# abeauvisage/uasl_motion_estimation

Measured on AMD Instinct MI355X. Metric: frames/sec + BA iter/sec, 2000 feats x 20-keyframe window, 1/2/4/8 MI355X, higher is better.
Workload: dtype u8+f32 (MI), f64 (BA); 1 GPU; config 3: 1280x720 stereo, 2000 feats, 20-keyframe window, 11x11 MI patches; frame=KLT + MI scale LM (LM, MAX_NB_ITER 10, tolerances off) + 10 BA LM iterations, parallelism=1 independent streams (one per GPU)

## Files before the change

uasl_motion_estimation_amd/csrc/ba.hip:

```cpp
#include <algorithm>
#include <cmath>
#include <cstdio>
#include <cstring>
#include <mutex>
#include <numeric>
#include <vector>
#include <hip/hip_ext.h>
#include "me_internal.hpp"
#include "ba_kernels.hpp"
#include "roster.hpp"
#include "solve_diag.hpp"
#include "me_device.hpp"

using me_dev::wave_sync;

using namespace ba;

namespace {

constexpr double kDblMin = 2.2250738585072014e-308;
constexpr double kDblEps = 2.220446049250313e-16;

template <int Ctrl>
__device__ __forceinline__ double dpp_f64(double x);
// ... 196 lines not shown
    *rho0 = s;
    *sqrt_rho1 = 1.0;
  }
}

template <bool SC1>
__device__ __forceinline__ double a_ld(const double* p) {
  if (!SC1) return *p;
  return __builtin_bit_cast(double, __hip_atomic_load(reinterpret_cast<const unsigned long long*>(p), ME_HO_LD,
                                                      __HIP_MEMORY_SCOPE_AGENT));
}
template <bool SC1>
__device__ __forceinline__ void a_st(double* p, double v) {
  if (!SC1) {
    *p = v;
    return;
  }
  __hip_atomic_store(reinterpret_cast<unsigned long long*>(p), __builtin_bit_cast(unsigned long long, v),
                     ME_HO_ST, __HIP_MEMORY_SCOPE_AGENT);
}
__device__ __forceinline__ void drain_and_barrier() {
  asm volatile("s_waitcnt vmcnt(0)" ::: "memory");
  __syncthreads();
}


constexpr int kPtBlock = 64;

#ifndef ME_LIN_SMALL
#define ME_LIN_SMALL 64
#endif
constexpr int kLinSmall = ME_LIN_SMALL, kLinSmallMaxObs = 64 * 512;
__host__ __device__ inline int lin_block(int no) { return no <= kLinSmallMaxObs ? kLinSmall : kBlock; }
template <int OD, int BLK>
__global__ __launch_bounds__(BLK) void linearize_kernel(Geo g, Bufs b) {
  __shared__ double lds[BLK / 64];
  const State* st = b.st;
  if (st->done || !st->need_lin) return;
  const int o = blockIdx.x * BLK + threadIdx.x;
  double cost = 0;
  if (o < g.no) {
    const int cur = st->cur;
    const int ci = b.cam_idx[o], pi = b.pt_idx[o];
    double r[4], Jc[24], Jp[12];
    obs_residual<OD>(g, b, o, b.cams[cur] + 6 * ci, b.pts[cur] + 3 * pi, r, Jc, Jp);
    const double s = r[0] * r[0] + r[1] * r[1] + r[2] * r[2] + r[3] * r[3];
    double rho0, sc;
    huber(s, &rho0, &sc);
    cost = 0.5 * rho0;
    for (int k = 0; k < 4; ++k) r[k] *= sc;
    for (int k = 0; k < 24; ++k) Jc[k] *= sc;
    for (int k = 0; k < 12; ++k) Jp[k] *= sc;
    const long slot = b.pos[o];
    double* X = b.obsx + slot * kObsxStride;
    X[0] = Jp[0] * Jp[0] + Jp[3] * Jp[3] + Jp[6] * Jp[6] + Jp[9] * Jp[9];
    X[1] = Jp[0] * Jp[1] + Jp[3] * Jp[4] + Jp[6] * Jp[7] + Jp[9] * Jp[10];
    X[2] = Jp[0] * Jp[2] + Jp[3] * Jp[5] + Jp[6] * Jp[8] + Jp[9] * Jp[11];
    X[3] = Jp[1] * Jp[1] + Jp[4] * Jp[4] + Jp[7] * Jp[7] + Jp[10] * Jp[10];
    X[4] = Jp[1] * Jp[2] + Jp[4] * Jp[5] + Jp[7] * Jp[8] + Jp[10] * Jp[11];
    X[5] = Jp[2] * Jp[2] + Jp[5] * Jp[5] + Jp[8] * Jp[8] + Jp[11] * Jp[11];
    for (int a = 0; a < 3; ++a) X[6 + a] = Jp[a] * r[0] + Jp[3 + a] * r[1] + Jp[6 + a] * r[2] + Jp[9 + a] * r[3];
    if (ci - g.nf >= 0) {
      double* W = b.Wo + 18 * slot;
      for (int a = 0; a < 6; ++a)
        for (int c = 0; c < 3; ++c)
          W[a * 3 + c] = Jc[a] * Jp[c] + Jc[6 + a] * Jp[3 + c] + Jc[12 + a] * Jp[6 + c] + Jc[18 + a] * Jp[9 + c];
    }
  }
  double v[1] = {cost};
  double out[1];
  block_sum<1>(v, out, lds);
  if (threadIdx.x == 0) b.part[R_COST * g.pstride + blockIdx.x] = out[0];
}

__device__ __forceinline__ bool last_arrival_wt(unsigned* cnt, unsigned expected) {
  __shared__ int slast;
  __syncthreads();
  if (threadIdx.x == 0) {
    asm volatile("s_waitcnt vmcnt(0)" ::: "memory");
    const unsigned k = __hip_atomic_fetch_add(cnt, 1u, ME_HO_RMW, __HIP_MEMORY_SCOPE_AGENT);
    slast = k == expected - 1;
    if (slast) __hip_atomic_store(cnt, 0u, __ATOMIC_RELAXED, __HIP_MEMORY_SCOPE_AGENT);
  }
  __syncthreads();
  return slast != 0;
}

__device__ void cam_reduce_body(const Geo& g, const Bufs& b, int sharded, const double* cpart, double* colnorm,
                                double* gc_raw, double* Uraw, int ci, int first, int count) {
  __shared__ double tot[27];
  __shared__ double csl[6];
  const State* st = b.st;
  const int u = threadIdx.x;
  if (u < 27) {
    double sum = 0.0;
    for (int k = 0; k < count; ++k) sum += a_ld<true>(&cpart[27 * ((long)first + k) + u]);
    tot[u] = sum;
    if (u < 21) Uraw[21 * (long)ci + u] = sum;
    else gc_raw[6 * ci + u - 21] = sum;
  }
// ... 164 lines not shown
  double d0 = A[0];
  if (!(d0 > 0)) return false;
  d0 = sqrt(d0);
  const double l10 = A[3] / d0, l20 = A[6] / d0;
  double d1 = A[4] - l10 * l10;
  if (!(d1 > 0)) return false;
  d1 = sqrt(d1);
  const double l21 = (A[7] - l20 * l10) / d1;
  double d2 = A[8] - l20 * l20 - l21 * l21;
  if (!(d2 > 0)) return false;
  d2 = sqrt(d2);
  L[0] = d0; L[1] = 0; L[2] = 0;
  L[3] = l10; L[4] = d1; L[5] = 0;
  L[6] = l20; L[7] = l21; L[8] = d2;
  return true;
}
__device__ __forceinline__ void fwd3(const double* L, const double* b, double* y) {
  y[0] = b[0] / L[0];
  y[1] = (b[1] - L[3] * y[0]) / L[4];
  y[2] = (b[2] - L[6] * y[0] - L[7] * y[1]) / L[8];
}
__device__ __forceinline__ void bwd3(const double* L, const double* y, double* x) {
  x[2] = y[2] / L[8];
  x[1] = (y[1] - L[7] * x[2]) / L[4];
  x[0] = (y[0] - L[3] * x[1] - L[6] * x[2]) / L[0];
}

constexpr int kSchurPts = 16, kSchurPtsWide = 32, kSchurPtsSmall = 8;
#ifndef ME_SCHUR_NT
#define ME_SCHUR_NT 5
#endif
constexpr int kSchurNtMax = ME_SCHUR_NT;
constexpr size_t kSchurLdsCap = 150 * 1024;
__host__ __device__ inline size_t schur_lds_bytes(int P, int Rz) { return 8 * (size_t)3 * P * Rz + 4 * 3 * (size_t)P; }

template <int W>
__device__ __forceinline__ int group_min(int x) {
  if (W >= 2) x = min(x, dpp_i32<kDppQuadSwap1>(x));
  if (W >= 4) x = min(x, dpp_i32<kDppQuadSwap2>(x));
  if (W >= 8) x = min(x, dpp_i32<kDppRowHalfMirror>(x));
  if (W >= 16) x = min(x, dpp_i32<kDppRowMirror>(x));
  if (W >= 32) x = min(x, __shfl_xor(x, 16, W));
  if (W >= 64) x = min(x, __shfl_xor(x, 32, W));
  return x;
}
template <int W>
__device__ __forceinline__ int group_max(int x) {
  if (W >= 2) x = max(x, dpp_i32<kDppQuadSwap1>(x));
  if (W >= 4) x = max(x, dpp_i32<kDppQuadSwap2>(x));
  if (W >= 8) x = max(x, dpp_i32<kDppRowHalfMirror>(x));
  if (W >= 16) x = max(x, dpp_i32<kDppRowMirror>(x));
  if (W >= 32) x = max(x, __shfl_xor(x, 16, W));
  if (W >= 64) x = max(x, __shfl_xor(x, 32, W));
  return x;
}

#ifdef ME_SCHUR_STAMPS
#define SCHUR_T(i)                                                                     \
  do {                                                                                 \
    if (sblk == 0 && threadIdx.x == 0) {                                               \
      const long long tt_ = (long long)__builtin_amdgcn_s_memtime();                   \
      if ((i) > 0) st->stamps[5 + (i)] += tt_ - sch_prev_;                             \
      sch_prev_ = tt_;                                                                 \
    }                                                                                  \
  } while (0)
#else
#define SCHUR_T(i) \
  do {             \
  } while (0)
#endif
template <int NT, int BLK, int PTS>
__global__ __launch_bounds__(BLK) void pt_schur_kernel(Geo g, Bufs b, Opts o, CamArgs ca) {
  constexpr int SL = BLK / PTS, NW = BLK / 64;
  extern __shared__ double smem[];
  __shared__ double red[8];
  if (ca.on && (int)blockIdx.x < ca.ncam) {
    if (threadIdx.x >= kBlock) return;
    const int q = blockIdx.x;
    if (q >= g.ncu) return;
#ifdef ME_EXP_NOCAM
    return;
#endif
    if (g.od == 4)
      cam_assemble_body<4>(g, b, ca.cpart, 0, ca.colnorm, ca.gc_raw, ca.Uraw, q);
    else
      cam_assemble_body<2>(g, b, ca.cpart, 0, ca.colnorm, ca.gc_raw, ca.Uraw, q);
    return;
  }
  const int sblk = (int)blockIdx.x - (ca.on ? ca.ncam : 0);
  State* st = b.st;
  if (st->done) return;
#ifdef ME_SCHUR_STAMPS
  long long sch_prev_ = 0;
  if (sblk == 0 && threadIdx.x == 0) st->stamps[12] += 1;
#endif
  SCHUR_T(0);
  const int need_lin = st->need_lin, scaled = st->scaled, cur = st->cur;
  const double* obsx = b.obsx;
  const double* Wo = b.Wo;
  const double radius = st->radius;
  const bool final_pass = st->iterations >= o.max_num_iterations;
  if (sblk == 0 && threadIdx.x == 0) st->final_pass = final_pass;
  const int P = g.spts, Rz = g.Rpad, rows = 3 * P, nks = rows / 4;
  const int sup = sblk / (8 * g.sgrp), r8 = sblk - sup * 8 * g.sgrp;
  const int run = 8 * sup + (r8 & 7), tgrp = r8 >> 3;
  if (run >= g.nruns) {
    if (need_lin && threadIdx.x == 0) b.part[R_GMAX_PT * g.pstride + sblk] = 0.0;
    return;
  }
  const int bA = g.sorted ? b.rband[2 * run] : 0, bB = g.sorted ? b.rband[2 * run + 1] : g.T - 1;
  const int nb = bB - bA + 1, ns = nb + (bB < g.T - 1 ? 1 : 0), ntile = ns * (ns + 1) / 2;
  if (tgrp * g.stpw >= ntile) {
    if (need_lin && threadIdx.x == 0) b.part[R_GMAX_PT * g.pstride + sblk] = 0.0;
    return;
  }
  const bool lead = tgrp == 0;
  double* Y = smem;
  int* band = reinterpret_cast<int*>(Y + (size_t)rows * Rz);
  const int tid = threadIdx.x, lane = tid & 63, wave = __builtin_amdgcn_readfirstlane(tid >> 6);
  const int gi = tid / SL, gl = tid & (SL - 1);
  int tI[NT], tJ[NT];
#pragma unroll
  for (int u = 0; u < NT; ++u) {
    int p = tgrp * g.stpw + wave + NW * u, ka = 0;
    if (p >= ntile) p = -1;
    int rem = p < 0 ? 0 : p;
    while (rem >= ns - ka) {
      rem -= ns - ka;
      ++ka;
    }
    const int kb = ka + rem;
    tI[u] = p < 0 ? -1 : (ka < nb ? bA + ka : g.T - 1);
    tJ[u] = p < 0 ? -1 : (kb < nb ? bA + kb : g.T - 1);
  }
  double4_t acc[NT];
#pragma unroll
  for (int u = 0; u < NT; ++u) acc[u] = double4_t{0.0, 0.0, 0.0, 0.0};
  double gm = 0;
  for (int sc = 0; sc < g.rsub; ++sc) {
    const int pos = run * g.rlen + sc * P + gi;
    const int j = pos < g.np ? (g.sorted ? b.order[pos] : pos) : g.np;
    double* Yp = Y + (size_t)(3 * gi) * Rz;
    for (int i = gl; i < 3 * Rz / 2; i += SL) reinterpret_cast<double2*>(Yp)[i] = double2{0.0, 0.0};
    if (j < g.np) {
      const int beg = b.p_off[j], end = b.p_off[j + 1];
      const int q0 = beg + gl;
      int ci0 = -1, cprev0 = -1, cnext0 = -2;
      double w0[18], cs0[6], X0[9];
      for (int i = 0; i < 9; ++i) X0[i] = 0.0;
      if (q0 < end) {
        ci0 = b.p_cam[q0];
        if (q0 > beg) cprev0 = b.p_cam[q0 - 1];
        if (q0 + 1 < end) cnext0 = b.p_cam[q0 + 1];
        if (need_lin)
          for (int i = 0; i < 9; ++i) X0[i] = obsx[(long)q0 * kObsxStride + i];
        if (ci0 >= 0) {
          for (int i = 0; i < 18; ++i) w0[i] = Wo[18 * (long)q0 + i];
          for (int a = 0; a < 6; ++a) cs0[a] = b.csc[6 * ci0 + a];
        }
      }
      double Vs[9], gs[3], pv[3], xv[3];
      if (need_lin) {
        for (int a = 0; a < 3; ++a) xv[a] = b.pts[cur][3 * (long)j + a];
        if (scaled)
          for (int a = 0; a < 3; ++a) pv[a] = b.psc[3 * (long)j + a];
        double V[9];
        for (int i = 0; i < 9; ++i) V[i] = X0[i];
        for (int q = q0 + SL; q < end; q += SL)
          for (int i = 0; i < 9; ++i) V[i] += obsx[(long)q * kObsxStride + i];
        SCHUR_T(1);
      for (int i = 0; i < 9; ++i) V[i] = group_sum<SL>(V[i]);
        if (!scaled) {
          pv[0] = g.jacobi ? 1.0 / (1.0 + sqrt(V[0])) : 1.0;
          pv[1] = g.jacobi ? 1.0 / (1.0 + sqrt(V[3])) : 1.0;
          pv[2] = g.jacobi ? 1.0 / (1.0 + sqrt(V[5])) : 1.0;
        }
        const double p0 = pv[0], p1 = pv[1], p2 = pv[2];
        Vs[0] = V[0] * p0 * p0; Vs[1] = V[1] * p0 * p1; Vs[2] = V[2] * p0 * p2;
        Vs[3] = Vs[1];          Vs[4] = V[3] * p1 * p1; Vs[5] = V[4] * p1 * p2;
        Vs[6] = Vs[2];          Vs[7] = Vs[5];          Vs[8] = V[5] * p2 * p2;
        gs[0] = V[6] * p0;
        gs[1] = V[7] * p1;
        gs[2] = V[8] * p2;
        if (gl == 0 && lead) {
          if (!scaled)
            for (int a = 0; a < 3; ++a) b.psc[3 * (long)j + a] = pv[a];
          for (int i = 0; i < 9; ++i) b.V[9 * (long)j + i] = Vs[i];
          for (int a = 0; a < 3; ++a) b.gps[3 * (long)j + a] = gs[a];
          for (int a = 0; a < 3; ++a) {
            const double xp = fmin(fmax(xv[a] - V[6 + a], g.lo[a]), g.hi[a]);
            gm = fmax(gm, fabs(xv[a] - xp));
          }
        }
      } else {
        for (int i = 0; i < 9; ++i) Vs[i] = b.V[9 * (long)j + i];
        for (int a = 0; a < 3; ++a) {
          gs[a] = b.gps[3 * (long)j + a];
          pv[a] = b.psc[3 * (long)j + a];
        }
      }
      if (!final_pass) {
      double A[9], L[9], z[3];
// ... 109 lines not shown
        auto reads = [&](const double* Yr, double* a, double* bb) {
#pragma unroll
          for (int u = 0; u < NT; ++u) {
            a[u] = Yr[cI[u]];
            bb[u] = Yr[cJ[u]];
          }
        };
        double an[NT], bn[NT];
        reads(Y0, av, bv);
#pragma unroll 1
        for (int ks = 0; ks < NKS; ks += 2) {
          reads(Y0 + (ks + 1) * kstride, an, bn);
          __builtin_amdgcn_sched_barrier(0);
          contract(ks, av, bv);
          __builtin_amdgcn_sched_barrier(0);
          reads(Y0 + min(ks + 2, NKS - 1) * kstride, av, bv);
          __builtin_amdgcn_sched_barrier(0);
          contract(ks + 1, an, bn);
          __builtin_amdgcn_sched_barrier(0);
        }
      } else {
        for (int ks = 0; ks < nks; ++ks) {
          operands(ks, av, bv);
          contract(ks, av, bv);
        }
      }
    }
    __syncthreads();
  }
  SCHUR_T(4);
  if (need_lin) {
    const double r = block_max(gm, red);
    if (tid == 0) b.part[R_GMAX_PT * g.pstride + sblk] = r;
  }
  if (final_pass) return;
#pragma unroll
  for (int u = 0; u < NT; ++u) {
    const int p = tgrp * g.stpw + wave + NW * u;
    if (p >= ntile) continue;
    double* dst = b.Spart + ((long)run * g.npairs + p) * 256;
#pragma unroll
    for (int i = 0; i < 4; ++i) dst[((lane >> 4) + 4 * i) * 16 + (lane & 15)] = acc[u][i];
  }
#ifdef ME_SCHUR_STAMPS
  __builtin_amdgcn_s_waitcnt(0);
#endif
  SCHUR_T(5);
}

constexpr int kFinBlock = 256;
__device__ void lin_finalize_body(const Geo& g, const Bufs& b, const Opts& o, const double* gc_raw,
                                  double* lds ) {
  State* st = b.st;
  if (st->done) return;
  if (st->need_lin) {
    const bool x = b.xch != nullptr;
    const int t = threadIdx.x;
    const bool in = t < kFinBlock;
    double c = 0, m = 0;
    if (!x && in) {
      for (int i = t; i < g.nblk_lin; i += kFinBlock) c += b.part[R_COST * g.pstride + i];
      for (int i = t; i < g.ksplit; i += kFinBlock) m = fmax(m, b.part[R_GMAX_PT * g.pstride + i]);
    }
    const double* gcv = x ? b.xch + xo_gc(g) : gc_raw;
    if (in)
      for (int i = t; i < g.n6; i += kFinBlock) m = fmax(m, fabs(gcv[i]));
    if (x && in)
      for (int i = t; i < g.xslots; i += kFinBlock) m = fmax(m, b.xch[xo_gmax(g) + i]);
    double v[1] = {c}, out[1];
    block_sum<1>(v, out, lds, kFinBlock / 64);
    const double mm = block_max(m, lds + 8);
    if (threadIdx.x == 0) {
      st->x_cost = x ? b.xch[xo_cost(g)] : out[0];
      const double gm = mm;
      if (!st->scaled) {
        st->initial_cost = st->x_cost;
        st->scaled = 1;
      }
      st->need_lin = 0;
      if (gm <= o.gradient_tolerance) {
        st->done = 1;
        st->termination = 0;
      }
    }
    __syncthreads();
  }
  if (threadIdx.x != 0 || st->done) return;
  if (st->iterations >= o.max_num_iterations) {
    st->done = 1;
    st->termination = 1;
    return;
  }
  if (st->radius <= o.min_radius) {
    st->done = 1;
    st->termination = 0;
    return;
  }
  st->iterations += 1;
}

__global__ __launch_bounds__(kFinBlock) void lin_finalize_kernel(Geo g, Bufs b, Opts o, const double* gc_raw) {
  __shared__ double lds[16];
  lin_finalize_body(g, b, o, gc_raw, lds);
}

__device__ void xch_tail_body(const Geo& g, const Bufs& b, const double* gc_raw, double* lds ) {
  const State* st = b.st;
  double c = 0, m = 0;
  if (st->need_lin) {
    for (int i = threadIdx.x; i < g.nblk_lin; i += kFinBlock) c += b.part[R_COST * g.pstride + i];
    for (int i = threadIdx.x; i < g.ksplit; i += kFinBlock) m = fmax(m, b.part[R_GMAX_PT * g.pstride + i]);
  }
  double* x = b.xch;
  for (int i = threadIdx.x; i < g.n6; i += kFinBlock) x[xo_gc(g) + i] = gc_raw[i];
  for (int i = threadIdx.x; i < g.xslots; i += kFinBlock)
    if (i != g.xrank) x[xo_gmax(g) + i] = 0.0;
  double v[1] = {c}, out[1];
  block_sum<1>(v, out, lds);
  const double mm = block_max(m, lds + 8);
  if (threadIdx.x == 0) {
    x[xo_cost(g)] = out[0];
    x[xo_fail(g)] = st->fail ? 1.0 : 0.0;
    x[xo_gmax(g) + g.xrank] = mm;
  }
}

constexpr int kSaElems = 32, kSaGroups = kBlock / kSaElems;
__host__ __device__ inline int solve_ld(int Ts) { return ((16 * Ts + 31) / 32) * 32 + 2; }
enum { SA_SUM = 0, SA_PACK = 1, SA_UNPACK = 2 };
template <int NTH, bool SC1>
__device__ bool s_assemble_body(const Geo& g, const Bufs& b, int blk, int full, int mode = SA_SUM,
                                double* img = nullptr, const Opts* o = nullptr, unsigned* claim = nullptr,
                                unsigned gen = 0) {
  constexpr int EL = NTH / kSaGroups;
  __shared__ double part[kSaGroups][EL];
  __shared__ int s_claimed;
  unsigned claim_old = 0;
  if (claim && threadIdx.x == 0) claim_old = me_roster_dev::fetch_max(claim, gen);
  const State* st = b.st;
  const bool live = !(st->done || st->final_pass);
  const int n = g.n6;
  const int e = threadIdx.x % EL, grp = threadIdx.x / EL;
  const int idx = blk * EL + e;
// ... 1770 lines not shown
  }
}

__global__ __launch_bounds__(kBlock) void output_kernel(Geo g, Bufs b, double* cams_dst, double* pts_dst) {
  const int cur = b.st->cur;
  const long gid = (long)blockIdx.x * kBlock + threadIdx.x;
  constexpr int kStateWords = (int)(sizeof(State) / 8);
  if (gid < kStateWords) b.out[gid] = ((const double*)b.st)[gid];
  if (gid < 6 * (long)g.nc) cams_dst[gid] = b.cams[cur][gid];
  if (gid < 3 * (long)g.np) pts_dst[gid] = b.pts[cur][gid];
}

struct Plan {
  me_ctx* c = nullptr;
  Geo g;
  unsigned asm_gen = 0;
  Bufs b;
  Opts o;
  double* colnorm = nullptr;
  double* gc_raw = nullptr;
  double* Uraw = nullptr;
  double* cpart = nullptr;
  double* host = nullptr;
  State* hstate[2] = {nullptr, nullptr};
  bool dev = false;
  bool copy_out = false;
  bool reserve_only = false;
  size_t solve_lds = 0;
  size_t schur_lds = 0;
  int use_lds = 0;
  int solve_flags = 0;
  int n_enq = 0;
  bool no_fused_asm = false;
  bool full_S = false;
  int solve_cap = 0;
  me_comm* comm = nullptr;
  bool xmax_separate = false;
};

inline long rup(long x, long m) { return (x + m - 1) / m * m; }
int blocks(long n, int bs) { return (int)std::max(1L, (n + bs - 1) / bs); }

void schur_geometry(int npairs, int np, int Rpad, Geo& g) {
  const bool wide = schur_lds_bytes(kSchurPtsWide, Rpad) <= kSchurLdsCap;
  const bool split_wide = wide && npairs <= 40 && np <= 256 * kSchurPts;
  g.spts = wide ? kSchurPtsWide : npairs > 100 ? kSchurPtsSmall : kSchurPts;
  g.nsub = (int)std::max(1L, ((long)np + g.spts - 1) / g.spts);
  g.rsub = (int)std::max(1L, ((long)g.nsub + 255) / 256);
  g.rlen = g.spts * g.rsub;
  g.nruns = (int)std::max(1L, ((long)np + g.rlen - 1) / g.rlen);
  const int nt = split_wide ? 2 : npairs > 100 ? kSchurNtMax : std::min(kSchurNtMax, 4);
  g.stpw = 8 * std::min((npairs + 7) / 8, nt);
  g.sgrp = (npairs + g.stpw - 1) / g.stpw;
  g.ksplit = (g.sgrp > 1 ? (int)rup((long)g.nruns, 8) : g.nruns) * g.sgrp;
  g.sorted = npairs > 40 ? 1 : 0;
}

void ba_geometry(Geo& g, int n_cams, int fixed_frames, int n_pts) {
  g.nc = n_cams;
  g.np = n_pts;
  g.nf = std::min(std::max(fixed_frames, 0), n_cams);
  g.m = g.nc - g.nf;
  g.n6 = 6 * g.m;
  g.Rpad = (int)rup(g.n6 + 1, 16);
  g.T = g.Rpad / 16;
  g.Ts = (g.n6 + 1 + 15) / 16;
// ... 24 lines not shown
  ME_CHECK(c, p->n_cams > 0 && p->n_pts >= 0 && p->n_obs >= 0, "BA: bad sizes");
  ME_CHECK(c, p->n_cams <= kMaxScanCams, "BA: at most %d cameras per window", kMaxScanCams);
  ME_CHECK(c, p->obs_dim == 0 || p->obs_dim == 2 || p->obs_dim == 4, "BA: obs_dim must be 2 or 4 (Observation<M>)");
  const bool mono = p->obs_dim == 2;
  ME_CHECK(c, p->feat_var > 0 && (mono || p->baseline != 0.0), "BA: wrong calibration parameters (BundleAdjuster.h:147)");
  ME_CHECK(c, !mono || p->cam_id || p->n_obs == 0, "BA: obs_dim 2 needs cam_id (Observation::camID)");
  const double baseline = mono && p->baseline == 0 ? 0.5 : p->baseline;
  ME_CHECK(c, p->mem == ME_HOST || p->mem == ME_DEVICE, "BA: bad memory kind");
  if (p->mem == ME_HOST) {
    for (int i = 0; i < p->n_obs; ++i) {
      ME_CHECK(c, p->cam_idx[i] >= 0 && p->cam_idx[i] < p->n_cams && p->pt_idx[i] >= 0 && p->pt_idx[i] < p->n_pts,
               "BA: observation %d indexes outside the window", i);
    }
  }
  P.c = c;
  int hook = c->dbg_solve_flags;
  if ((hook & kFlagFailEveryOther) && (c->dbg_solve_count++ & 1)) hook |= kFlagSolveFail;
  P.no_fused_asm = (hook & kFlagSeparateAsm) != 0;
  P.solve_flags = hook & (kFlagAsmTimeout | kFlagSolveFail | kFlagRosterNow);
  Geo& g = P.g;
  ba_geometry(g, p->n_cams, p->fixed_frames, p->n_pts);
  g.no = p->n_obs;
  g.od = mono ? 2 : 4;
  P.comm = comm;
  P.xmax_separate = comm && comm->world == 0;
  g.xslots = comm && comm->world > 0 ? comm->world : 1;
  g.xrank = comm && comm->world > 0 ? comm->rank : 0;
  ME_CHECK(c, g.nruns <= kMaxRuns, "BA: %d Schur runs exceed %d", g.nruns, kMaxRuns);
  g.nblkp = blocks(std::max(g.np, 1), kBlock);
  ME_CHECK(c, g.npairs <= 8 * 24, "BA: %d variable cameras exceed the Schur tile budget", g.m);
  g.nblk_obs = (int)std::max(1L, rup(std::max(g.no, 1), kBlock) / kBlock);
  g.nblk_lin = (int)std::max(1L, rup(std::max(g.no, 1), lin_block(g.no)) / lin_block(g.no));
  g.nblk_pts = (int)std::max(1L, rup(std::max(g.np, 1), kPtBlock) / kPtBlock);
  g.jacobi = opt->jacobi_scaling ? 1 : 0;
  g.ncu = (int)(rup(std::max(g.no, 1), kBlock) / kBlock) + g.m;
  g.nblk_step = (int)std::max(1L, rup(std::max(g.np, 1), kStepPts) / kStepPts);
  g.pstride = std::max({g.nblk_obs, g.nblk_lin, g.nblk_pts, g.nblk_step, g.ksplit});
  std::memcpy(g.K0, p->K0, sizeof(g.K0));
  std::memcpy(g.K1, p->K1, sizeof(g.K1));
  g.baseline = baseline;
  g.sinv = 1.0 / std::sqrt(p->feat_var);
  const double Zmax = p->K0[0] * baseline / 0.1;
  const double Zmin = p->K0[0] * baseline / (2 * p->K0[2]);
  g.hi[0] = Zmax / p->K0[0] * p->K0[2];
  g.hi[1] = Zmax / p->K0[4] * p->K0[5];
  g.hi[2] = Zmax;
  g.lo[0] = -Zmax / p->K0[0] * p->K0[2];
  g.lo[1] = -Zmax / p->K0[4] * p->K0[5];
  g.lo[2] = Zmin;
  Opts& o = P.o;
  o.max_num_iterations = opt->max_num_iterations;
  o.function_tolerance = opt->function_tolerance;
  o.gradient_tolerance = opt->gradient_tolerance;
  o.parameter_tolerance = opt->parameter_tolerance;
  o.initial_radius = opt->initial_trust_region_radius;
  o.max_radius = opt->max_trust_region_radius;
  o.min_radius = opt->min_trust_region_radius;
  o.min_diag = opt->min_lm_diagonal;
  o.max_diag = opt->max_lm_diagonal;
  o.min_rel_decrease = opt->min_relative_decrease;
  o.max_invalid = opt->max_num_consecutive_invalid_steps;
  const bool dev = p->mem == ME_DEVICE;
  const long nb = g.pstride;
  Bufs& b = P.b;
  std::vector<std::pair<size_t, void**>> items;
  auto add = [&](size_t bytes, void* dst) { items.push_back({rup((long)std::max<size_t>(bytes, 8), 256), (void**)dst}); };
  add(8 * 6 * (size_t)g.nc, &b.cams[0]);
  add(8 * 3 * (size_t)g.np, &b.pts[0]);
  add(8 * g.od * (size_t)g.no, &b.obs);
  add(4 * (size_t)g.no, &b.cam_idx);
  add(4 * (size_t)g.no, &b.pt_idx);
  add(mono ? 4 * (size_t)g.no : 0, &b.cam_id);
  const size_t n_inputs = items.size();
  add(8 * 6 * (size_t)g.nc, &b.cams[1]);
  add(8 * 3 * (size_t)g.np, &b.pts[1]);
  add(4 * (size_t)(g.np + 1), &b.p_off);
  add(4 * (size_t)g.no, &b.p_obs);
  add(4 * (size_t)g.no, &b.pos);
  add(4 * (size_t)g.no, &b.p_cam);
  add(4 * (size_t)(g.m + 1), &b.c_off);
  add(4 * (size_t)g.no, &b.c_obs);
  add(4 * (size_t)g.no, &b.tmp_obs);
  add(4 * (size_t)g.no, &b.cpos);
  add(8 * kObsxStride * (size_t)g.no, &b.obsx);
  add((size_t)g.no, &b.dup);
  add(8 * solve_a_doubles(g.Ts), &b.Abuf);
  add(8 * 18 * (size_t)g.no, &b.Wo);
  add(8 * (size_t)g.n6, &b.csc);
  add(8 * 3 * (size_t)g.np, &b.psc);
  add(8 * 36 * (size_t)g.m, &b.U);
  add(8 * (size_t)g.n6, &b.gcs);
  add(8 * 9 * (size_t)g.np, &b.V);
  add(8 * 3 * (size_t)g.np, &b.gps);
  add(8 * 9 * (size_t)g.np, &b.Lp);
  add(8 * 3 * (size_t)g.np, &b.zp);
  add(8 * 256 * (size_t)g.nruns * g.npairs, &b.Spart);
  add(4 * (size_t)std::max(g.np, 1), &b.order);
  add(4 * (size_t)std::max(g.np, 1), &b.pkey);
  add(4 * (size_t)std::max(g.np, 1), &b.prank);
  add(4 * (size_t)g.T * g.T * g.nblkp, &b.phist);
  add(8 * (size_t)g.nruns, &b.rband);
  add(4 * (size_t)g.npairs * g.nruns, &b.tl);
  add(4 * (size_t)g.npairs, &b.tcnt);
  add(8 * (size_t)g.n6 * g.n6 + 8 * (size_t)(2 * g.n6 + 2), &b.S);
  add(8 * (size_t)g.n6, &b.yc);
  add(8 * 3 * (size_t)g.np, &b.dp);
  add(8 * R_COUNT * (size_t)nb, &b.part);
  add(8 * (R_COUNT + 2), &b.scal);
  add(sizeof(State), &b.st);
  add(8 * (size_t)(g.n6 + 2), &P.colnorm);
  add(8 * (size_t)g.n6, &P.gc_raw);
  add(8 * 21 * (size_t)std::max(g.m, 1), &P.Uraw);
  add(8 * 27 * (size_t)g.ncu, &P.cpart);
  add(4 * (size_t)kCuStride * (size_t)rup(g.ncu, 8), &b.cunit);
  add(4 * (size_t)(g.m + 1 + 3 + 2), &b.cnt);
  add(4 * (size_t)blocks((long)g.npairs * 256, kSolveBlock / kSaGroups), &b.asm_claim);
  const size_t work_bytes = 4 * (2 * (size_t)g.np + (size_t)g.nblk_obs * g.nc + 4);
// ... 45 lines not shown
    const size_t len[6] = {8 * 6 * (size_t)g.nc, 8 * 3 * (size_t)g.np, 8 * g.od * (size_t)g.no, 4 * (size_t)g.no,
                           4 * (size_t)g.no, mono ? 4 * (size_t)g.no : 0};
    size_t off = 0;
    for (int k = 0; k < 6; ++k) {
      if (len[k]) std::memcpy(h + off, src[k], len[k]);
      off += items[k].first;
    }
    ME_HIP(c, hipMemcpyAsync(b.cams[0], hp, input_span, hipMemcpyHostToDevice, s));
  } else {
    b.obs = p->obs;
    b.cam_idx = p->cam_idx;
    b.pt_idx = p->pt_idx;
    if (mono) b.cam_id = p->cam_id;
  }
  ME_HIP(c, hipMemsetAsync(b.cnt, 0, (size_t)((char*)b.work - (char*)b.cnt) + work_bytes, s));
  P.asm_gen = 0;
  const double* cams_in = dev ? p->cams : b.cams[0];
  const double* pts_in = dev ? p->pts : b.pts[0];
  const long nthr = std::max({(long)g.nblk_obs * kBlock, (long)g.np, 6L * g.nc, 3L * g.np});
  hipLaunchKernelGGL(plan_count_kernel, dim3(blocks(nthr, kBlock)), dim3(kBlock), 4 * (size_t)g.nc, s, g, b, cams_in,
                     pts_in);
  hipLaunchKernelGGL(plan_scan_kernel, dim3(1), dim3(kScanBlock), 0, s, g, b, o);
  hipLaunchKernelGGL(plan_scatter_kernel, dim3(g.nblk_obs), dim3(kBlock), 0, s, g, b);
  hipLaunchKernelGGL(plan_segsort_kernel, dim3(blocks(std::max(g.np, 1), kSortBlock / 64)), dim3(kSortBlock), 0, s, g,
                     b);
  if (g.sorted) {
    hipLaunchKernelGGL(plan_band_kernel, dim3(g.nblkp), dim3(kBlock), 0, s, g, b);
    hipLaunchKernelGGL(plan_order_kernel, dim3(1), dim3(kScanBlock), 0, s, g, b);
  }
  ME_TRY(me_check_launch(c, "BA plan"));
  P.use_lds = solve_form(g.Ts) == 0 ? 1 : 0;
  P.solve_lds = 8 * (solve_small_doubles(g.Ts) + (P.use_lds ? solve_a_doubles(g.Ts) : 0));
  ME_CHECK(c, P.solve_lds <= kSolveLdsCap, "BA: %d variable cameras exceed the camera-solve workspace", g.m);
  P.schur_lds = schur_lds_bytes(g.spts, g.Rpad);
  ME_CHECK(c, P.schur_lds <= kSchurLdsCap, "BA: %d variable cameras exceed the Schur workspace", g.m);
  if (!c->ba_lds_attr) {
    for (const void* k : {(const void*)cam_solve_kernel<0>, (const void*)cam_solve_kernel<1>, (const void*)cam_solve_kernel<2>})
      ME_HIP(c, hipFuncSetAttribute(k, hipFuncAttributeMaxDynamicSharedMemorySize, (int)kSolveLdsCap));
#define ME_SCHUR_K(N)                                                                                   \
  (const void*)pt_schur_kernel<N, 512, kSchurPts>, (const void*)pt_schur_kernel<N, 512, kSchurPtsWide>, \
      (const void*)pt_schur_kernel<N, 512, kSchurPtsSmall>
    for (const void* k : {ME_SCHUR_K(2), ME_SCHUR_K(3), ME_SCHUR_K(4), ME_SCHUR_K(5)})
#undef ME_SCHUR_K
      ME_HIP(c, hipFuncSetAttribute(k, hipFuncAttributeMaxDynamicSharedMemorySize, (int)kSchurLdsCap));
    c->ba_lds_attr = 1;
  }
  if (!P.use_lds) {
    int per_cu = 0;
    ME_HIP(c, hipOccupancyMaxActiveBlocksPerMultiprocessor(&per_cu, cam_solve_kernel<2>, kSolveBlock, P.solve_lds));
    P.solve_cap = std::max(0, per_cu) * (c->cu_active > 0 ? c->cu_active : c->num_cu);
    if (P.comm && g.Ts >= kSolveMwMinTs) {
      double* d = P.b.scal;
      const double v = -(double)P.solve_cap;
      ME_HIP(c, hipMemcpyAsync(d, &v, 8, hipMemcpyHostToDevice, c->stream));
      ME_TRY(me_comm_allreduce_impl(P.comm, d, 1, ME_COMM_MAX));
      double r = 0.0;
      ME_HIP(c, hipMemcpyAsync(&r, d, 8, hipMemcpyDeviceToHost, c->stream));
      ME_HIP(c, hipStreamSynchronize(c->stream));
      P.solve_cap = (int)-r;
    }
  }
  return ME_OK;
}



#define ME_XCH(ptr, n, op) ME_TRY(me_comm_allreduce_impl(P.comm, (ptr), (long)(n), (op)))

int enqueue_linearize(Plan& P) {
  me_ctx* c = P.c;
  const Geo& g = P.g;
  hipStream_t s = c->stream;
  const bool sh = P.comm != nullptr;
  {
    me_ktimer t(c, ME_KT_BA_LINEARIZE);
    const bool small = lin_block(g.no) == kLinSmall;
    if (g.od == 4 && small)
      hipLaunchKernelGGL((linearize_kernel<4, kLinSmall>), dim3(g.nblk_lin), dim3(kLinSmall), 0, s, g, P.b);
    else if (g.od == 4)
      hipLaunchKernelGGL((linearize_kernel<4, kBlock>), dim3(g.nblk_lin), dim3(kBlock), 0, s, g, P.b);
    else if (small)
      hipLaunchKernelGGL((linearize_kernel<2, kLinSmall>), dim3(g.nblk_lin), dim3(kLinSmall), 0, s, g, P.b);
    else
      hipLaunchKernelGGL((linearize_kernel<2, kBlock>), dim3(g.nblk_lin), dim3(kBlock), 0, s, g, P.b);
  }
  const bool first = P.n_enq == 0;
  const bool fused = !first && g.m > 0;
  ++P.n_enq;
  CamArgs ca{P.cpart, P.colnorm, P.gc_raw, P.Uraw, fused ? 1 : 0, fused ? (g.ncu + 7) / 8 * 8 : 0};
  if (g.m > 0 && !fused)
    hipLaunchKernelGGL(cam_assemble_kernel, dim3(g.ncu), dim3(kBlock), 0, s, g, P.b, P.cpart, sh ? 1 : 0,
                       P.colnorm, P.gc_raw, P.Uraw);
  if (sh && !fused) {
    if (first) {
      hipLaunchKernelGGL(xch_flags_kernel, dim3(1), dim3(1), 0, s, g, P.b, P.colnorm);
      ME_XCH(P.colnorm, g.n6 + 2, ME_COMM_SUM);
    }
    hipLaunchKernelGGL(cam_finish_kernel, dim3(blocks(std::max(g.m, 1), 64)), dim3(64), 0, s, g, P.b,
                       (const double*)P.colnorm, (const double*)P.gc_raw, (const double*)P.Uraw, first ? 1 : 0);
  }
  {
    me_ktimer t(c, ME_KT_BA_SCHUR, true);
    const int pw8 = g.stpw / 8;
    const dim3 grd(g.ksplit + ca.ncam);
#define ME_SCHUR(N)                                                                                          \
  do {                                                                                                       \
    if (g.spts == kSchurPtsWide)                                                                             \
      hipExtLaunchKernelGGL((pt_schur_kernel<N, 512, kSchurPtsWide>), grd, dim3(512), P.schur_lds, s, t.a, t.b, 0, g, \
                            P.b, P.o, ca);                                                                   \
    else if (g.spts == kSchurPtsSmall)                                                                       \
      hipExtLaunchKernelGGL((pt_schur_kernel<N, 512, kSchurPtsSmall>), grd, dim3(512), P.schur_lds, s, t.a, t.b, 0, g, \
                            P.b, P.o, ca);                                                                   \
    else                                                                                                     \
      hipExtLaunchKernelGGL((pt_schur_kernel<N, 512, kSchurPts>), grd, dim3(512), P.schur_lds, s, t.a, t.b, 0, g, P.b, \
                            P.o, ca);                                                                        \
  } while (0)
    static_assert(kSchurNtMax >= 3 && kSchurNtMax <= 5, "instantiated tile counts");
    if (pw8 <= 2) ME_SCHUR(2);
    else if (pw8 <= 3) ME_SCHUR(3);
    else if (pw8 <= 4) ME_SCHUR(4);
    else ME_SCHUR(5);
#undef ME_SCHUR
  }
  if (sh) {
    hipLaunchKernelGGL(s_assemble_kernel, dim3(blocks((long)g.npairs * 256, kSaElems) + 1), dim3(kBlock), 0, s, g,
                       P.b, P.o, (const double*)P.gc_raw, 0, (int)SA_PACK);
    if (P.xmax_separate) {
      ME_XCH(P.b.xch, xo_gmax(g), ME_COMM_SUM);
      ME_XCH(P.b.xch + xo_gmax(g), 1, ME_COMM_MAX);
    } else {
      ME_XCH(P.b.xch, xo_total(g), ME_COMM_SUM);
    }
  }
  return me_check_launch(c, "BA linearize");
}

int enqueue_assemble(Plan& P, bool img = false) {
  me_ctx* c = P.c;
  const Geo& g = P.g;
  const int mode = P.comm ? SA_UNPACK : SA_SUM;
  if (g.m > 0)
    hipLaunchKernelGGL(s_assemble_kernel, dim3(blocks((long)g.npairs * 256, kSaElems) + 1), dim3(kBlock), 0,
                       c->stream, g, P.b, P.o, (const double*)P.gc_raw, P.full_S ? 1 : 0, mode,
                       img && !P.full_S ? P.b.Abuf : nullptr);
  else
    hipLaunchKernelGGL(lin_finalize_kernel, dim3(1), dim3(kFinBlock), 0, c->stream, g, P.b, P.o,
                       (const double*)P.gc_raw);
  return me_check_launch(c, "BA assemble");
}

int enqueue_iteration(Plan& P, bool last = false) {
  me_ctx* c = P.c;
  const Geo& g = P.g;
  hipStream_t s = c->stream;
  const bool sh = P.comm != nullptr;
// ... 712 lines not shown
```

uasl_motion_estimation_amd/csrc/ba_kernels.hpp:

```cpp
#pragma once
#include <hip/hip_runtime.h>
#include <stdint.h>

namespace ba {

typedef double double4_t __attribute__((ext_vector_type(4)));

constexpr int kBlock = 256;
constexpr int kObsxStride = 9;

struct Opts {
  int max_num_iterations;
  double function_tolerance, gradient_tolerance, parameter_tolerance;
  double initial_radius, max_radius, min_radius, min_diag, max_diag, min_rel_decrease;
  int max_invalid;
};

struct State {
  int cur;
  int need_lin;
  int done;
  int termination;
  int iterations, successful, invalid_count;
  int fail;
  int scaled;
  int accepted;
  int bad_input;
  int infeasible;
  int final_pass;
  int spin_err;
  int pad[2];
  double radius, decrease;
  double x_cost, cand_cost, model_change, initial_cost;
  double cam_step2, cam_xn2, cam_model;
  double last_q;
  long long stamps[16];
};

enum { R_COST = 0, R_GMAX_PT, R_MODEL, R_CAND, R_STEP2, R_XN2, R_COUNT };

struct Geo {
  int nc, np, no, nf, m, n6, Rpad, T, Ts, spts, nsub, ksplit, npairs, nblk_obs, nblk_lin, nblk_pts, nblk_step, pstride, jacobi,
      ncu;
  int nruns, rlen, rsub, sgrp, stpw, nblkp;
  int sorted;
  int od;
  int xslots, xrank;
  double K0[9], K1[9];
  double baseline, sinv;
  double lo[3], hi[3];
};

struct Bufs {
  double* cams[2];
  double* pts[2];
  const double* obs;
  const int* cam_idx;
  const int* pt_idx;
  const int* cam_id;
  int* p_off;
  int* p_obs;
  int* pos;
  int* p_cam;
  int* c_off;
  int* c_obs;
  int* tmp_obs;
  int* cpos;
  int* cunit;
  double* obsx;
  uint8_t* dup;
  double* Abuf;
  double* Wo;
  double* csc;
  double* psc;
  double* U;
  double* gcs;
  double* V;
  double* gps;
  double* Lp;
// ... 38 lines not shown
```

Baseline: 1360 frames/s.

## Fuse BA linearization into the point Schur kernel when geometry allows

When the Schur configuration fits (small tile count, unsorted runs, single subrun, enough LDS), each Schur block now computes residuals, Jacobians and Huber weighting for its own points' observations. It accumulates the per-point 3x3 blocks in LDS instead of writing them to a global obsx buffer and reading them back. The separate linearize kernel launch and the obsx allocation are skipped, and per-run cost partials replace the per-block linearize partials. In exchange the kernel is instantiated per observation dimension, uses extra LDS (which may lower occupancy), and serialises the per-slot accumulation with repeated block-wide barriers.

```diff
diff --git a/uasl_motion_estimation_amd/csrc/ba.hip b/uasl_motion_estimation_amd/csrc/ba.hip
--- a/uasl_motion_estimation_amd/csrc/ba.hip
+++ b/uasl_motion_estimation_amd/csrc/ba.hip
@@ -252,6 +252,31 @@
 #endif
 constexpr int kLinSmall = ME_LIN_SMALL, kLinSmallMaxObs = 64 * 512;
 __host__ __device__ inline int lin_block(int no) { return no <= kLinSmallMaxObs ? kLinSmall : kBlock; }
+template <int OD>
+__device__ __forceinline__ double lin_pieces(const Geo& g, const Bufs& b, long o, const double* cam, const double* pt,
+                                             bool var, double* X, double* W) {
+  double r[4], Jc[24], Jp[12];
+  obs_residual<OD>(g, b, o, cam, pt, r, Jc, Jp);
+  const double s = r[0] * r[0] + r[1] * r[1] + r[2] * r[2] + r[3] * r[3];
+  double rho0, sc;
+  huber(s, &rho0, &sc);
+  for (int k = 0; k < 4; ++k) r[k] *= sc;
+  for (int k = 0; k < 24; ++k) Jc[k] *= sc;
+  for (int k = 0; k < 12; ++k) Jp[k] *= sc;
+  X[0] = Jp[0] * Jp[0] + Jp[3] * Jp[3] + Jp[6] * Jp[6] + Jp[9] * Jp[9];
+  X[1] = Jp[0] * Jp[1] + Jp[3] * Jp[4] + Jp[6] * Jp[7] + Jp[9] * Jp[10];
+  X[2] = Jp[0] * Jp[2] + Jp[3] * Jp[5] + Jp[6] * Jp[8] + Jp[9] * Jp[11];
+  X[3] = Jp[1] * Jp[1] + Jp[4] * Jp[4] + Jp[7] * Jp[7] + Jp[10] * Jp[10];
+  X[4] = Jp[1] * Jp[2] + Jp[4] * Jp[5] + Jp[7] * Jp[8] + Jp[10] * Jp[11];
+  X[5] = Jp[2] * Jp[2] + Jp[5] * Jp[5] + Jp[8] * Jp[8] + Jp[11] * Jp[11];
+  for (int a = 0; a < 3; ++a) X[6 + a] = Jp[a] * r[0] + Jp[3 + a] * r[1] + Jp[6 + a] * r[2] + Jp[9 + a] * r[3];
+  if (var)
+    for (int a = 0; a < 6; ++a)
+      for (int c = 0; c < 3; ++c)
+        W[a * 3 + c] = Jc[a] * Jp[c] + Jc[6 + a] * Jp[3 + c] + Jc[12 + a] * Jp[6 + c] + Jc[18 + a] * Jp[9 + c];
+  return 0.5 * rho0;
+}
+
 template <int OD, int BLK>
 __global__ __launch_bounds__(BLK) void linearize_kernel(Geo g, Bufs b) {
   __shared__ double lds[BLK / 64];
@@ -262,30 +287,9 @@
   if (o < g.no) {
     const int cur = st->cur;
     const int ci = b.cam_idx[o], pi = b.pt_idx[o];
-    double r[4], Jc[24], Jp[12];
-    obs_residual<OD>(g, b, o, b.cams[cur] + 6 * ci, b.pts[cur] + 3 * pi, r, Jc, Jp);
-    const double s = r[0] * r[0] + r[1] * r[1] + r[2] * r[2] + r[3] * r[3];
-    double rho0, sc;
-    huber(s, &rho0, &sc);
-    cost = 0.5 * rho0;
-    for (int k = 0; k < 4; ++k) r[k] *= sc;
-    for (int k = 0; k < 24; ++k) Jc[k] *= sc;
-    for (int k = 0; k < 12; ++k) Jp[k] *= sc;
     const long slot = b.pos[o];
-    double* X = b.obsx + slot * kObsxStride;
-    X[0] = Jp[0] * Jp[0] + Jp[3] * Jp[3] + Jp[6] * Jp[6] + Jp[9] * Jp[9];
-    X[1] = Jp[0] * Jp[1] + Jp[3] * Jp[4] + Jp[6] * Jp[7] + Jp[9] * Jp[10];
-    X[2] = Jp[0] * Jp[2] + Jp[3] * Jp[5] + Jp[6] * Jp[8] + Jp[9] * Jp[11];
-    X[3] = Jp[1] * Jp[1] + Jp[4] * Jp[4] + Jp[7] * Jp[7] + Jp[10] * Jp[10];
-    X[4] = Jp[1] * Jp[2] + Jp[4] * Jp[5] + Jp[7] * Jp[8] + Jp[10] * Jp[11];
-    X[5] = Jp[2] * Jp[2] + Jp[5] * Jp[5] + Jp[8] * Jp[8] + Jp[11] * Jp[11];
-    for (int a = 0; a < 3; ++a) X[6 + a] = Jp[a] * r[0] + Jp[3 + a] * r[1] + Jp[6 + a] * r[2] + Jp[9 + a] * r[3];
-    if (ci - g.nf >= 0) {
-      double* W = b.Wo + 18 * slot;
-      for (int a = 0; a < 6; ++a)
-        for (int c = 0; c < 3; ++c)
-          W[a * 3 + c] = Jc[a] * Jp[c] + Jc[6 + a] * Jp[3 + c] + Jc[12 + a] * Jp[6 + c] + Jc[18 + a] * Jp[9 + c];
-    }
+    cost = lin_pieces<OD>(g, b, o, b.cams[cur] + 6 * ci, b.pts[cur] + 3 * pi, ci - g.nf >= 0,
+                          b.obsx + slot * kObsxStride, b.Wo + 18 * slot);
   }
   double v[1] = {cost};
   double out[1];
@@ -516,7 +520,23 @@
 #endif
 constexpr int kSchurNtMax = ME_SCHUR_NT;
 constexpr size_t kSchurLdsCap = 150 * 1024;
+constexpr size_t kSchurLinLds = 8 * 9 * 512;
 __host__ __device__ inline size_t schur_lds_bytes(int P, int Rz) { return 8 * (size_t)3 * P * Rz + 4 * 3 * (size_t)P; }
+
+#ifndef ME_SCHUR_FUSED_NT
+#define ME_SCHUR_FUSED_NT 4
+#endif
+__host__ __device__ constexpr bool schur_fused_lin(int od, int nt, int pts) {
+  return (od == 4 || od == 2) && nt <= ME_SCHUR_FUSED_NT && (nt <= 3 || (nt == 4 && pts != kSchurPtsSmall));
+}
+__host__ __device__ constexpr int schur_nt(int stpw) {
+  return stpw / 8 <= 2 ? 2 : stpw / 8 <= 3 ? 3 : stpw / 8 <= 4 ? 4 : 5;
+}
+
+__device__ __forceinline__ void own_stores_visible() {
+  __builtin_amdgcn_fence(__ATOMIC_RELEASE, "workgroup");
+  __builtin_amdgcn_fence(__ATOMIC_ACQUIRE, "workgroup");
+}
 
 template <int W>
 __device__ __forceinline__ int group_min(int x) {
@@ -553,9 +573,10 @@
   do {             \
   } while (0)
 #endif
-template <int NT, int BLK, int PTS>
+template <int OD, int NT, int BLK, int PTS>
 __global__ __launch_bounds__(BLK) void pt_schur_kernel(Geo g, Bufs b, Opts o, CamArgs ca) {
   constexpr int SL = BLK / PTS, NW = BLK / 64;
+  constexpr bool FL = schur_fused_lin(OD, NT, PTS);
   extern __shared__ double smem[];
   __shared__ double red[8];
   if (ca.on && (int)blockIdx.x < ca.ncam) {
@@ -565,10 +586,7 @@
 #ifdef ME_EXP_NOCAM
     return;
 #endif
-    if (g.od == 4)
-      cam_assemble_body<4>(g, b, ca.cpart, 0, ca.colnorm, ca.gc_raw, ca.Uraw, q);
-    else
-      cam_assemble_body<2>(g, b, ca.cpart, 0, ca.colnorm, ca.gc_raw, ca.Uraw, q);
+    cam_assemble_body<OD>(g, b, ca.cpart, 0, ca.colnorm, ca.gc_raw, ca.Uraw, q);
     return;
   }
   const int sblk = (int)blockIdx.x - (ca.on ? ca.ncam : 0);
@@ -603,6 +621,42 @@
   int* band = reinterpret_cast<int*>(Y + (size_t)rows * Rz);
   const int tid = threadIdx.x, lane = tid & 63, wave = __builtin_amdgcn_readfirstlane(tid >> 6);
   const int gi = tid / SL, gl = tid & (SL - 1);
+  const bool flin = FL && g.flin && need_lin;
+  double* vl = reinterpret_cast<double*>(band + 3 * P);
+  __shared__ double cwave[NW];
+  if constexpr (FL) {
+    if (flin) {
+      const int j0 = run * g.rlen;
+      const int s0 = b.p_off[j0], s1 = b.p_off[min(j0 + P, g.np)];
+      double cost = 0;
+      for (int base = s0; base < s1; base += BLK) {
+        const int q = base + tid;
+        int k = -1, cell = 0;
+        double X[9];
+        if (q < s1) {
+          const int ob = b.p_obs[q], ci = b.p_cam[q];
+          const int j = b.pt_idx[ob];
+          const int beg = b.p_off[j];
+          double xl[3], w[18];
+          for (int a = 0; a < 3; ++a) xl[a] = b.pts[cur][3 * (long)j + a];
+          const bool var = ci >= 0 && !final_pass;
+          cost += lin_pieces<OD>(g, b, ob, b.cams[cur] + 6 * (ci + g.nf), xl, var, X, w);
+          if (var)
+            for (int i = 0; i < 18; ++i) b.Wo[18 * (long)q + i] = w[i];
+          k = (q - beg) / SL;
+          cell = 9 * ((j - j0) * SL + ((q - beg) & (SL - 1)));
+        }
+        own_stores_visible();
+        for (int r = 0;; ++r) {
+          if (k == r)
+            for (int i = 0; i < 9; ++i) vl[cell + i] = r == 0 ? X[i] : vl[cell + i] + X[i];
+          if (!__syncthreads_or(k > r)) break;
+        }
+      }
+      cost = wave_total(cost);
+      if (lane == 0) cwave[wave] = cost;
+    }
+  }
   int tI[NT], tJ[NT];
 #pragma unroll
   for (int u = 0; u < NT; ++u) {
@@ -636,7 +690,7 @@
         ci0 = b.p_cam[q0];
         if (q0 > beg) cprev0 = b.p_cam[q0 - 1];
         if (q0 + 1 < end) cnext0 = b.p_cam[q0 + 1];
-        if (need_lin)
+        if (need_lin && !flin)
           for (int i = 0; i < 9; ++i) X0[i] = obsx[(long)q0 * kObsxStride + i];
         if (ci0 >= 0) {
           for (int i = 0; i < 18; ++i) w0[i] = Wo[18 * (long)q0 + i];
@@ -649,9 +703,13 @@
         if (scaled)
           for (int a = 0; a < 3; ++a) pv[a] = b.psc[3 * (long)j + a];
         double V[9];
-        for (int i = 0; i < 9; ++i) V[i] = X0[i];
-        for (int q = q0 + SL; q < end; q += SL)
-          for (int i = 0; i < 9; ++i) V[i] += obsx[(long)q * kObsxStride + i];
+        if (flin) {
+          for (int i = 0; i < 9; ++i) V[i] = q0 < end ? vl[9 * tid + i] : 0.0;
+        } else {
+          for (int i = 0; i < 9; ++i) V[i] = X0[i];
+          for (int q = q0 + SL; q < end; q += SL)
+            for (int i = 0; i < 9; ++i) V[i] += obsx[(long)q * kObsxStride + i];
+        }
         SCHUR_T(1);
       for (int i = 0; i < 9; ++i) V[i] = group_sum<SL>(V[i]);
         if (!scaled) {
@@ -827,6 +885,11 @@
   if (need_lin) {
     const double r = block_max(gm, red);
     if (tid == 0) b.part[R_GMAX_PT * g.pstride + sblk] = r;
+    if (flin && lead && tid == 0) {
+      double c = 0;
+      for (int w = 0; w < NW; ++w) c += cwave[w];
+      b.part[R_COST * g.pstride + run] = c;
+    }
   }
   if (final_pass) return;
 #pragma unroll
@@ -854,7 +917,7 @@
     const bool in = t < kFinBlock;
     double c = 0, m = 0;
     if (!x && in) {
-      for (int i = t; i < g.nblk_lin; i += kFinBlock) c += b.part[R_COST * g.pstride + i];
+      for (int i = t; i < g.ncost; i += kFinBlock) c += b.part[R_COST * g.pstride + i];
       for (int i = t; i < g.ksplit; i += kFinBlock) m = fmax(m, b.part[R_GMAX_PT * g.pstride + i]);
     }
     const double* gcv = x ? b.xch + xo_gc(g) : gc_raw;
@@ -903,7 +966,7 @@
   const State* st = b.st;
   double c = 0, m = 0;
   if (st->need_lin) {
-    for (int i = threadIdx.x; i < g.nblk_lin; i += kFinBlock) c += b.part[R_COST * g.pstride + i];
+    for (int i = threadIdx.x; i < g.ncost; i += kFinBlock) c += b.part[R_COST * g.pstride + i];
     for (int i = threadIdx.x; i < g.ksplit; i += kFinBlock) m = fmax(m, b.part[R_GMAX_PT * g.pstride + i]);
   }
   double* x = b.xch;
@@ -2740,6 +2803,7 @@
   int solve_flags = 0;
   int n_enq = 0;
   bool no_fused_asm = false;
+  bool fused_lin = false;
   bool full_S = false;
   int solve_cap = 0;
   me_comm* comm = nullptr;
@@ -2830,6 +2894,10 @@
   g.nblk_obs = (int)std::max(1L, rup(std::max(g.no, 1), kBlock) / kBlock);
   g.nblk_lin = (int)std::max(1L, rup(std::max(g.no, 1), lin_block(g.no)) / lin_block(g.no));
   g.nblk_pts = (int)std::max(1L, rup(std::max(g.np, 1), kPtBlock) / kPtBlock);
+  P.fused_lin = schur_fused_lin(g.od, schur_nt(g.stpw), g.spts) && g.rsub == 1 && !g.sorted &&
+                (g.sgrp == 1 || g.ksplit <= 128) && schur_lds_bytes(g.spts, g.Rpad) + kSchurLinLds <= kSchurLdsCap;
+  g.flin = P.fused_lin ? 1 : 0;
+  g.ncost = P.fused_lin ? g.nruns : g.nblk_lin;
   g.jacobi = opt->jacobi_scaling ? 1 : 0;
   g.ncu = (int)(rup(std::max(g.no, 1), kBlock) / kBlock) + g.m;
   g.nblk_step = (int)std::max(1L, rup(std::max(g.np, 1), kStepPts) / kStepPts);
@@ -2880,7 +2948,7 @@
   add(4 * (size_t)g.no, &b.c_obs);
   add(4 * (size_t)g.no, &b.tmp_obs);
   add(4 * (size_t)g.no, &b.cpos);
-  add(8 * kObsxStride * (size_t)g.no, &b.obsx);
+  add(P.fused_lin ? 0 : 8 * kObsxStride * (size_t)g.no, &b.obsx);
   add((size_t)g.no, &b.dup);
   add(8 * solve_a_doubles(g.Ts), &b.Abuf);
   add(8 * 18 * (size_t)g.no, &b.Wo);
@@ -2992,15 +3060,16 @@
   P.use_lds = solve_form(g.Ts) == 0 ? 1 : 0;
   P.solve_lds = 8 * (solve_small_doubles(g.Ts) + (P.use_lds ? solve_a_doubles(g.Ts) : 0));
   ME_CHECK(c, P.solve_lds <= kSolveLdsCap, "BA: %d variable cameras exceed the camera-solve workspace", g.m);
-  P.schur_lds = schur_lds_bytes(g.spts, g.Rpad);
+  P.schur_lds = schur_lds_bytes(g.spts, g.Rpad) + (P.fused_lin ? kSchurLinLds : 0);
   ME_CHECK(c, P.schur_lds <= kSchurLdsCap, "BA: %d variable cameras exceed the Schur workspace", g.m);
   if (!c->ba_lds_attr) {
     for (const void* k : {(const void*)cam_solve_kernel<0>, (const void*)cam_solve_kernel<1>, (const void*)cam_solve_kernel<2>})
       ME_HIP(c, hipFuncSetAttribute(k, hipFuncAttributeMaxDynamicSharedMemorySize, (int)kSolveLdsCap));
-#define ME_SCHUR_K(N)                                                                                   \
-  (const void*)pt_schur_kernel<N, 512, kSchurPts>, (const void*)pt_schur_kernel<N, 512, kSchurPtsWide>, \
-      (const void*)pt_schur_kernel<N, 512, kSchurPtsSmall>
-    for (const void* k : {ME_SCHUR_K(2), ME_SCHUR_K(3), ME_SCHUR_K(4), ME_SCHUR_K(5)})
+#define ME_SCHUR_K(D, N)                                                                                      \
+  (const void*)pt_schur_kernel<D, N, 512, kSchurPts>, (const void*)pt_schur_kernel<D, N, 512, kSchurPtsWide>, \
+      (const void*)pt_schur_kernel<D, N, 512, kSchurPtsSmall>
+    for (const void* k : {ME_SCHUR_K(4, 2), ME_SCHUR_K(4, 3), ME_SCHUR_K(4, 4), ME_SCHUR_K(4, 5), ME_SCHUR_K(2, 2),
+                          ME_SCHUR_K(2, 3), ME_SCHUR_K(2, 4), ME_SCHUR_K(2, 5)})
 #undef ME_SCHUR_K
       ME_HIP(c, hipFuncSetAttribute(k, hipFuncAttributeMaxDynamicSharedMemorySize, (int)kSchurLdsCap));
     c->ba_lds_attr = 1;
@@ -3032,7 +3101,7 @@
   const Geo& g = P.g;
   hipStream_t s = c->stream;
   const bool sh = P.comm != nullptr;
-  {
+  if (!P.fused_lin) {
     me_ktimer t(c, ME_KT_BA_LINEARIZE);
     const bool small = lin_block(g.no) == kLinSmall;
     if (g.od == 4 && small)
@@ -3063,24 +3132,28 @@
     me_ktimer t(c, ME_KT_BA_SCHUR, true);
     const int pw8 = g.stpw / 8;
     const dim3 grd(g.ksplit + ca.ncam);
-#define ME_SCHUR(N)                                                                                          \
-  do {                                                                                                       \
-    if (g.spts == kSchurPtsWide)                                                                             \
-      hipExtLaunchKernelGGL((pt_schur_kernel<N, 512, kSchurPtsWide>), grd, dim3(512), P.schur_lds, s, t.a, t.b, 0, g, \
-                            P.b, P.o, ca);                                                                   \
-    else if (g.spts == kSchurPtsSmall)                                                                       \
-      hipExtLaunchKernelGGL((pt_schur_kernel<N, 512, kSchurPtsSmall>), grd, dim3(512), P.schur_lds, s, t.a, t.b, 0, g, \
-                            P.b, P.o, ca);                                                                   \
-    else                                                                                                     \
-      hipExtLaunchKernelGGL((pt_schur_kernel<N, 512, kSchurPts>), grd, dim3(512), P.schur_lds, s, t.a, t.b, 0, g, P.b, \
-                            P.o, ca);                                                                        \
+#define ME_SCHUR_P(D, N, PTS) \
+  hipExtLaunchKernelGGL((pt_schur_kernel<D, N, 512, PTS>), grd, dim3(512), P.schur_lds, s, t.a, t.b, 0, g, P.b, P.o, ca)
+#define ME_SCHUR_D(D, N)                                                \
+  do {                                                                  \
+    if (g.spts == kSchurPtsWide) ME_SCHUR_P(D, N, kSchurPtsWide);       \
+    else if (g.spts == kSchurPtsSmall) ME_SCHUR_P(D, N, kSchurPtsSmall); \
+    else ME_SCHUR_P(D, N, kSchurPts);                                   \
+  } while (0)
+#define ME_SCHUR(N)                 \
+  do {                              \
+    if (g.od == 4) ME_SCHUR_D(4, N); \
+    else ME_SCHUR_D(2, N);          \
   } while (0)
     static_assert(kSchurNtMax >= 3 && kSchurNtMax <= 5, "instantiated tile counts");
+    static_assert(schur_nt(16) == 2 && schur_nt(24) == 3 && schur_nt(32) == 4 && schur_nt(40) == 5, "schur_nt is this dispatch");
     if (pw8 <= 2) ME_SCHUR(2);
     else if (pw8 <= 3) ME_SCHUR(3);
     else if (pw8 <= 4) ME_SCHUR(4);
     else ME_SCHUR(5);
 #undef ME_SCHUR
+#undef ME_SCHUR_D
+#undef ME_SCHUR_P
   }
   if (sh) {
     hipLaunchKernelGGL(s_assemble_kernel, dim3(blocks((long)g.npairs * 256, kSaElems) + 1), dim3(kBlock), 0, s, g,
diff --git a/uasl_motion_estimation_amd/csrc/ba_kernels.hpp b/uasl_motion_estimation_amd/csrc/ba_kernels.hpp
--- a/uasl_motion_estimation_amd/csrc/ba_kernels.hpp
+++ b/uasl_motion_estimation_amd/csrc/ba_kernels.hpp
@@ -45,6 +45,8 @@
   int nruns, rlen, rsub, sgrp, stpw, nblkp;
   int sorted;
   int od;
+  int flin;
+  int ncost;
   int xslots, xrank;
   double K0[9], K1[9];
   double baseline, sinv;
```

Measured after the change: 1378 frames/s (median of 6 runs). 1.3% higher.
